# xu-ji/IIC

Measured on AMD Instinct MI355X. Metric: paired-images/sec, STL10 96x96 ClusterNet5g+IID_loss, higher is better.
Workload: dtype bf16; 1 GPU; STL10 96x96 ClusterNet5g IID+ (cluster_sobel.py train step), batch 660 pairs/GPU, 5 sub-heads, k=70, bf16 MFMA convs / fp32 stem+heads+loss, fused HIP Adam; global_batch_pairs=660, input=96x96x1 grey -> sobel 2ch, parallelism=dp1, streams=2, launch=hip-graph replay: 6 linear graph segments, the two views on two streams

## Files before the change

iic_amd/_lib.py:

```python
import ctypes
import os
from ctypes import POINTER, Structure, c_double, c_float, c_int, c_int32, c_long, c_longlong, c_void_p

_HERE = os.path.dirname(os.path.abspath(__file__))
HAS_HOOKS = os.environ.get("IIC_HIP_LIB", "") == "dbg"
LIB_PATH = os.path.join(_HERE, "libiic_hip_dbg.so" if HAS_HOOKS else "libiic_hip.so")

IIC_MAX_TAPS = 32
IIC_STAT_STRIPES = 32


class ConvGeom(Structure):
  _fields_ = [
    ("N", c_int32), ("MY", c_int32), ("MX", c_int32),
    ("in_Hp", c_int32), ("in_Wp", c_int32), ("Cin", c_int32),
    ("sy", c_int32), ("sx", c_int32), ("oy", c_int32), ("ox", c_int32),
    ("out_Hp", c_int32), ("out_Wp", c_int32), ("Cout", c_int32),
    ("ty", c_int32), ("tx", c_int32), ("py", c_int32), ("px", c_int32),
    ("ntaps", c_int32),
    ("tap_off", c_int32 * IIC_MAX_TAPS),
    ("tap_w", c_int32 * IIC_MAX_TAPS),
    ("NP", c_int32),
    ("NP256", c_int32),
    ("NP64", c_int32),
    ("MP", c_int32),
  ]


_P = c_void_p
_SIGNATURES = {
  "iic_version": (c_int, []),
  "iic_iid_nsplit": (c_int, [c_int]),
  "iic_iid_workspace_bytes": (c_long, [c_int, c_int]),
  "iic_iid_joint_raw": (c_int, [_P, _P, _P, c_int, c_int, c_int, c_long, c_long, c_int, _P]),
  "iic_iid_loss_from_joint": (c_int, [_P, c_int, c_int, c_int, c_double, c_double, _P, _P, _P, _P, _P, _P]),
  "iic_iid_grad": (c_int, [_P, _P, _P, _P, _P, _P, _P, _P, c_int, c_int, c_int, c_long, c_long, _P]),
  "iic_seg_joint_nsplit": (c_int, [c_int, c_int, c_int, c_int]),
  "iic_seg_joint_raw": (c_int, [_P, _P, _P, _P, _P, c_int, c_int, c_int, c_int, c_int, c_int, _P]),
  "iic_seg_loss_from_joint": (c_int, [_P, c_int, c_int, c_int, c_double, c_double, _P, _P, _P, _P, _P, c_int, _P]),
  "iic_seg_grad_workspace_bytes": (c_long, [c_int, c_int]),
  "iic_seg_grad": (c_int, [_P, _P, _P, _P, _P, _P, _P, _P, c_int, c_int, c_int, c_int, c_int, c_int, c_int, _P, _P]),
  "iic_affine_warp_fwd": (c_int, [_P, _P, _P, c_int, c_int, c_int, c_int, c_int, c_int, _P]),
  "iic_affine_warp_bwd": (c_int, [_P, _P, _P, c_int, c_int, c_int, c_int, c_int, c_int, _P]),
  "iic_conv_lds_bytes": (c_long, [POINTER(ConvGeom), c_int]),
  "iic_conv_igemm": (c_int, [POINTER(ConvGeom), _P, _P, _P, _P, _P, _P, c_int, _P]),
  "iic_conv_wgrad_nsplit": (c_int, [POINTER(ConvGeom)]),
  "iic_conv_wgrad": (c_int, [POINTER(ConvGeom), _P, _P, _P, c_int, c_int, _P]),
  "iic_conv_wgrad_reduce": (c_int, [_P, c_int, c_int, c_int, c_int, _P, c_int, _P]),
  "iic_weight_prep": (c_int, [_P, _P, _P, c_int, c_int, c_int, _P]),
  "iic_conv_igemm_frag_supported": (c_int, [POINTER(ConvGeom)]),
  "iic_conv_igemm_frag": (c_int, [POINTER(ConvGeom), _P, _P, _P, _P, _P, _P, c_int, _P]),
  "iic_conv_igemm_red_supported": (c_int, [POINTER(ConvGeom)]),
  "iic_conv_igemm_frag_red": (c_int, [POINTER(ConvGeom), _P, _P, _P, _P, _P, _P, c_int, _P, _P, _P, _P, _P, _P]),
  "iic_weight_prep_frag": (c_int, [_P, _P, c_int, c_int, c_int, c_int, _P]),
  "iic_weight_prep_multi_blocks": (c_long, [c_int, c_int, c_int]),
  "iic_weight_prep_multi": (c_int, [_P, c_int, c_long, _P]),
  "iic_bn_finalize": (c_int, [_P, _P, _P, _P, _P, _P, _P, c_int, c_long, c_long, c_float, c_float, c_int, _P]),
  "iic_stat_bytes": (c_long, [c_int]),
  "iic_bn_running_update": (c_int, [c_int, POINTER(_P), POINTER(_P), POINTER(_P), POINTER(_P), POINTER(c_int),
                                    c_float, _P]),
  "iic_bn_apply": (c_int, [_P, _P, _P, _P, _P, _P, c_int, c_int, c_int, c_int, c_int, c_int, _P]),
  "iic_bn_bwd_reduce": (c_int, [_P, _P, _P, _P, _P, _P, _P, c_int, c_int, c_int, c_int, c_int, _P]),
  "iic_bn_bwd_finalize": (c_int, [_P, _P, _P, _P, _P, _P, c_int, c_long, _P]),
  "iic_bn_bwd_apply": (c_int, [_P, _P, _P, _P, _P, _P, _P, _P, _P, c_int, c_int, c_int, c_int, c_int, _P]),
  "iic_stem_stats": (c_int, [_P, _P, _P, c_int, c_int, c_int, c_int, _P]),
  "iic_stem_apply_pool": (c_int, [_P, _P, _P, _P, c_int, c_int, c_int, c_int, _P]),
  "iic_stem_bwd_reduce": (c_int, [_P, _P, _P, _P, _P, c_int, c_int, c_int, c_int, _P]),
  "iic_stem_wgrad_partial_floats": (c_long, []),
  "iic_stem_bwd_wgrad": (c_int, [_P, _P, _P, _P, _P, _P, _P, c_int, c_int, c_int, c_int, _P]),
  "iic_contingency": (c_int, [_P, _P, c_long, c_int, c_int, _P, _P]),
  "iic_count_equal": (c_int, [_P, _P, c_long, _P, _P]),
  "iic_augment": (c_int, [_P, c_int, c_int, c_int, c_int, _P, _P, c_int, _P, c_int, _P, _P, c_int, _P, _P, c_int, _P, _P]),
  "iic_seg_augment": (c_int, [_P, c_int, c_int, c_int, c_int, _P, _P, _P, _P, c_int, c_int, c_int, c_int, _P, _P, _P, _P,
                              _P, _P]),
  "iic_stem_bwd_fused": (c_int, [_P, _P, _P, _P, _P, _P, POINTER(c_int), c_int, c_int, c_int, c_int, _P]),
  "iic_stem_wgrad_combine": (c_int, [_P, c_int, _P, _P, c_int, _P]),
  "iic_firstconv_fwd": (c_int, [_P, _P, _P, _P, c_int, c_int, c_int, c_int, c_int, c_int, c_int, _P]),
  "iic_firstconv_wgrad_partial_floats": (c_long, []),
  "iic_firstconv_wgrad": (c_int, [_P, _P, _P, _P, c_int, c_int, c_int, c_int, c_int, c_int, c_int, _P]),
  "iic_maxpool2_fwd": (c_int, [_P, _P, c_int, c_int, c_int, c_int, c_int, c_int, _P]),
  "iic_maxpool2_bwd": (c_int, [_P, _P, _P, c_int, c_int, c_int, c_int, c_int, c_int, _P]),
  "iic_bn_relu_maxpool2_fwd": (c_int, [_P, _P, _P, c_int, c_int, c_int, c_int, c_int, c_int, _P]),
  "iic_bn_relu_maxpool2_bwd": (c_int, [_P, _P, _P, _P, c_int, c_int, c_int, c_int, c_int, c_int, _P]),
  "iic_sobel": (c_int, [_P, _P, c_int, c_int, c_int, c_int, c_int, c_int, _P]),
  "iic_avgpool_fwd": (c_int, [_P, _P, c_int, c_int, c_int, c_int, c_int, _P]),
# ... 100 lines not shown
```

iic_amd/archs/cluster.py:

```python
import torch
import torch.nn as nn

from .. import geom as G
from .. import ops

__all__ = ["ClusterNet5g", "ClusterNet5gTwoHead"]

import os
import weakref

from ..dist import SHARD_INPUTS, shard_batch
DEDUP = [int(os.environ.get("IIC_DEDUP", "1"))]
_ASSERTED_REPLICAS = [1]


class replicated(object):

  def __init__(self, r):
    self.r = int(r)

  def __enter__(self):
    self.prev = _ASSERTED_REPLICAS[0]
    _ASSERTED_REPLICAS[0] = self.r
    return self
# ... 194 lines not shown
      dy = ops.pt_alloc(N, H, W, 64, 1, dev)
      ops.bn_bwd_apply(da, None, y, bcoef, dy, N, H, W, 1, 64, mask_coef=coef)
      gf, _ = h.geoms(N, H, W)
      dW = ops.conv_wgrad(gf, xp, dy, 9).view(64, C, 3, 3)
    for t in (dpool, da, dy, xp, y, a):
      ops.POOL.release(t)
    return None, dW, dgamma, dbeta, None


class _BlockFn(torch.autograd.Function):
  @staticmethod
  def forward(ctx, x, w1, g1, b1, w2, g2, b2, wd, gd, bd, blk, chain=None):
    N, Hp, Wp, Cin = x.shape
    H, W = Hp - 2, Wp - 2
    dev = x.device
    h1, h2, hd = blk._h1, blk._h2, blk._hd
    planes = h1.spec.cout
    Ho, Wo = h1.spec.out_size(H), h1.spec.out_size(W)
    cnt = N * Ho * Wo
    need_grad = any(ctx.needs_input_grad)

    def bn_coef(bn, holder, gamma, beta, y_stats):
      rm, rv, nbt = _bn_buffers(bn)
      if _bn_training(bn):
        upd = bn.training
        return ops.bn_finalize(y_stats, gamma.detach(), beta.detach(), rm if upd else None,
                               rv if upd else None, nbt if upd else None, planes, cnt, True)
      return ops.bn_finalize(None, gamma.detach(), beta.detach(), rm, rv, None, planes, cnt, False)

    gf1, _ = h1.geoms(N, H, W)
    gf2, _ = h2.geoms(N, Ho, Wo)
    st1 = h1.stats(dev) if _bn_training(blk.bn1) else None
    y1 = ops.pt_alloc(N, Ho, Wo, planes, 1, dev)
    ops.conv_igemm(gf1, x, h1.weights()[0], y1, stats=st1)
    coef1 = bn_coef(blk.bn1, h1, g1, b1, st1)
    st2 = h2.stats(dev) if _bn_training(blk.bn2) else None
    y2 = ops.pt_alloc(N, Ho, Wo, planes, 1, dev)
    a1 = ops.pt_alloc(N, Ho, Wo, planes, 1, dev)
    ops.bn_apply(y1, coef1, a1, N, Ho, Wo, 1, planes, relu=True)
    ops.conv_igemm(gf2, a1, h2.weights()[0], y2, stats=st2)
    coef2 = bn_coef(blk.bn2, h2, g2, b2, st2)
    out = ops.pt_alloc(N, Ho, Wo, planes, 1, dev)
    yd = coefd = None
    if hd is not None:
      gfd, _ = hd.geoms(N, H, W)
      bnd = blk.downsample[1]
      std = hd.stats(dev) if _bn_training(bnd) else None
      yd = ops.pt_alloc(N, Ho, Wo, planes, 1, dev)
      ops.conv_igemm(gfd, x, hd.weights()[0], yd, stats=std)
      coefd = bn_coef(bnd, hd, gd, bd, std)
      ops.bn_apply(y2, coef2, out, N, Ho, Wo, 1, planes, y2=yd, coef2=coefd, relu=True)
    else:
      ops.bn_apply(y2, coef2, out, N, Ho, Wo, 1, planes, res=x, relu=True)

    if need_grad:
      ctx.blk = blk
      ctx.branch, ctx.pt_dtype = ops.BRANCH[0], ops.PT_DTYPE[0]
      ctx.dims = (N, H, W, Ho, Wo, Cin, planes)
      ctx.bn_batch = (_bn_training(blk.bn1) and _bn_training(blk.bn2))
      ctx.dout_premasked, ctx.mask_dx = blk._dout_premasked, blk._mask_dx
      ctx.dout_prereduced = False
      ctx.red_prev = None
      if chain is not None:
        _, gb1f = h1.geoms(N, H, W)
        if (chain.ctx is not None and FUSE_RED[0] and hd is None and blk._mask_dx and len(gb1f) == 1
            and ops.red_supported(gb1f[0], h1.weights()[1]) and ctx.bn_batch):
          ctx.red_prev = (chain.y2, chain.yd, chain.blk)
          chain.ctx.dout_prereduced = True
        if blk._dout_premasked and ctx.bn_batch:
          chain.ctx, chain.y2, chain.yd, chain.blk = ctx, y2, yd, blk
        else:
          chain.ctx = None
      ctx.save_for_backward(x, y1, a1, y2, out, yd, coef1, coef2, coefd, g1, g2, gd)
    else:
      if chain is not None:
        chain.ctx = None
      for t in (y1, a1, y2, yd):
        if t is not None:
          ops.POOL.release(t)
    return out

  @ops.branch_backward
# ... 31 lines not shown
      gfd, _ = hd.geoms(N, H, W)
      dWd = ops.conv_wgrad(gfd, x, dyd, 1, use_tr).view(planes, Cin, 1, 1)
    da1 = ops.pt_alloc(N, Ho, Wo, planes, 1, dev)
    s1 = h1.stats(dev, "bwd")
    m_act, m_coef = (None, coef1) if BN_MASK_FROM_Y[0] else (a1, None)
    w2b = h2.weights()[1]
    if FUSE_RED[0] and m_coef is not None and len(gb2) == 1 and ops.red_supported(gb2[0], w2b):
      ops.conv_igemm(gb2[0], dy2, w2b, da1, red=(y1, coef1, s1, None, None))
    else:
      for g in gb2:
        ops.conv_igemm(g, dy2, w2b, da1)
      ops.bn_bwd_reduce(da1, m_act, y1, s1, N, Ho, Wo, 1, planes, mask_coef=m_coef)
    bc1, dg1, db1 = ops.bn_bwd_finalize(s1, g1.detach(), coef1, planes, cnt)
    dy1 = ops.pt_alloc(N, Ho, Wo, planes, 1, dev)
    ops.bn_bwd_apply(da1, m_act, y1, bc1, dy1, N, Ho, Wo, 1, planes, mask_coef=m_coef)

    dW1 = ops.conv_wgrad(gf1, x, dy1, 9, use_tr).view(planes, Cin, 3, 3)
    dx = ops.pt_alloc(N, H, W, Cin, 1, dev)
    mx = x if mask_dx else None
    red_prev = None
    if ctx.red_prev is not None:
      py2, pyd, pblk = ctx.red_prev
      red_prev = (py2, None, pblk._h2.stats(dev, "bwd"), pyd,
                  pblk._hd.stats(dev, "bwd") if pyd is not None else None)
    if hd is None:
      for g in gb1:
        if pre or mask_dx:
          assert pre, "a block that pre-masks its input gradient needs a pre-masked output gradient"
          ops.conv_igemm(g, dy1, h1.weights()[1], dx, res_grad=dout, res_act=mx, premask=True,
                         red=red_prev)
        else:
          ops.conv_igemm(g, dy1, h1.weights()[1], dx, res_grad=dout, res_act=out)
    else:
      for g in gb1:
        ops.conv_igemm(g, dy1, h1.weights()[1], dx, res_act=mx, premask=mask_dx)
      _, gbd = hd.geoms(N, H, W)
      for g in gbd:
        ops.conv_igemm(g, dyd, hd.weights()[1], dx, accumulate=True, res_act=mx, premask=mask_dx)

    for t in (dout, dy2, dyd, da1, dy1, y1, a1, y2, yd, out):
      ops.POOL.release(t)
    return dx, dW1, dg1, db1, dW2, dg2, db2, dWd, dgd, dbd, None, None


APPLY_GENERATION = [0]


class _ApplyCounter(object):
  def _apply(self, fn, *a, **k):
    APPLY_GENERATION[0] += 1
    return super(_ApplyCounter, self)._apply(fn, *a, **k)


class BasicBlock(nn.Module):
  expansion = 1

  def __init__(self, inplanes, planes, stride=1, downsample=None, track_running_stats=None):
    super(BasicBlock, self).__init__()
    assert track_running_stats is not None
    self.conv1 = nn.Conv2d(inplanes, planes, kernel_size=3, stride=stride, padding=1, bias=False)
    self.bn1 = nn.BatchNorm2d(planes, track_running_stats=track_running_stats)
    self.conv2 = nn.Conv2d(planes, planes, kernel_size=3, stride=1, padding=1, bias=False)
    self.bn2 = nn.BatchNorm2d(planes, track_running_stats=track_running_stats)
    self.downsample = downsample
    self.stride = stride
    self._h1 = _ConvHolder(self.conv1)
    self._h2 = _ConvHolder(self.conv2)
    self._hd = _ConvHolder(downsample[0]) if downsample is not None else None
    self._use_tr = True
    self._dout_premasked = False
    self._mask_dx = False
# ... 241 lines not shown
```

iic_amd/csrc/conv_igemm_bd.hip:

```cpp
#include "common.h"
#include "conv_tile.h"
#include "../../include/iic_hip.h"

__device__ __forceinline__ void bd_bload(u32x4& d, const unsigned char* p) {
  asm volatile("global_load_dwordx4 %0, %1, off" : "=v"(d) : "v"(p) : "memory");
}
template <int N>
__device__ __forceinline__ void bd_bwait(u32x4& d) {
  asm volatile("s_waitcnt vmcnt(%1)" : "+v"(d) : "i"(N) : "memory");
}

struct bd_blk {
  int bw, bh, nbx, nby;
  int PW, npix, mul;
};

#define BD_BM 256
#define BD_BN 128
#define BD_THREADS 256
#define BD_PROF_SLOTS 16
#ifndef BD_STORE_UB
#define BD_STORE_UB 8
#endif

template <bool GATHER, int ABL, int MS, int RED, int WN = 2>
__device__ __forceinline__ void bd_tile(
    const iic_conv_geom& g, const bf16_t* __restrict__ in, const unsigned char* __restrict__ wfrag,
    bf16_t* __restrict__ out, float* __restrict__ stats, const bf16_t* __restrict__ res_grad,
    const bf16_t* __restrict__ res_act, int accumulate, int lds_a_bytes,
    const bf16_t* __restrict__ red_y, const float* __restrict__ red_coef,
    const bf16_t* __restrict__ red_y2, float* __restrict__ red_stats, float* __restrict__ red_stats2,
    unsigned long long* __restrict__ prof, int blk_in_class, int nwg_class, const bd_blk& B) {
  constexpr int BNT = WN * 64, NWM = 4 / WN;
  constexpr bool CANBLK = !GATHER && MS * 32 * (4 / WN) == 256;
  const bool blk = CANBLK && B.bw > 0;
  constexpr int CLD = BNT + 8;
  constexpr bool PROF = (ABL & 128) != 0;
  constexpr bool NEWORD = (ABL & 256) == 0;
  constexpr bool SWZ = (ABL & 512) == 0;
  unsigned long long t_stamp[8];
  unsigned long long t_bsum = 0, t_b0 = 0;
  int t_nb = 0;
  if (PROF) t_stamp[0] = __builtin_readcyclecounter();
  constexpr int BM = MS * 32 * NWM, WR = MS * 32;
  extern __shared__ __attribute__((aligned(16))) unsigned char smem_raw[];
  unsigned char* sA = smem_raw;
  int* s_pin = reinterpret_cast<int*>(smem_raw + lds_a_bytes);
  int* s_pout = s_pin + BM;
  float* s_red = reinterpret_cast<float*>(s_pout + BM);
  unsigned char* s_key = reinterpret_cast<unsigned char*>(s_red + NWM * 2 * BNT);
  bf16_t* sC = reinterpret_cast<bf16_t*>(smem_raw);

  const int tid = threadIdx.x, lane = tid & 63;
  const int wave = __builtin_amdgcn_readfirstlane(tid >> 6);
  const int wm = WN == 2 ? wave >> 1 : wave, wn = WN == 2 ? wave & 1 : 0;
  const int l31 = lane & 31, g5 = lane >> 5;

  const int nt = g.Cout / BNT;
  const int tix = xcd_tile_index(blk_in_class, nwg_class);
  const int mtile = tix / nt, ntile = tix - mtile * nt;
  const int n0 = ntile * BNT;
  const int m0 = mtile * BM;
  const int in_pixels = g.N * g.in_Hp * g.in_Wp;

  int v_tapoff = g.tap_off[lane & (IIC_MAX_TAPS - 1)];
// ... 29 lines not shown
  const int keyw = blk ? B.PW : g.in_Wp;
  const int jskip = blk ? B.PW - B.bw
                        : ((!GATHER && g.sx == 1 && ((g.in_Wp - g.MX) & 1) == 0) ? g.in_Wp - g.MX : 0);
  auto dense_of = [&](int p) { return p - jskip * (p / keyw); };
  int arow[MS];
  int drow[MS];
#pragma unroll
  for (int ms = 0; ms < MS; ++ms) {
    const int row = wm * WR + ms * 32 + l31;
    const int pr = GATHER ? row : (s_pin[row] - p_lo);
    arow[ms] = SWZ ? pr : pr * ROWB + g5 * 16;
    drow[ms] = (SWZ && !GATHER) ? dense_of(s_pin[row]) : pr;
  }
  if (!GATHER && jskip != 0) {
    for (int r = tid; r < npix; r += BD_THREADS) s_key[r] = (unsigned char)((dense_of(p_lo + r) >> 1) & 7);
    __syncthreads();
  }
  const int v_tapd = v_tapoff - jskip * (v_tapoff / keyw);
  const int nblk = (npix * 128 + 1023) >> 10;
  auto dma_patch = [&](int c0) {
    for (int kb = wave; kb < nblk; kb += BD_THREADS / 64) {
      const int q = kb * 64 + lane;
      const int r = q >> 3;
      const int ls = (q & 7) ^ (GATHER ? ((r >> 1) & 7)
                                       : (jskip != 0 ? (int)s_key[r < npix ? r : npix - 1]
                                                     : (((p_lo + r) >> 1) & 7)));
      long p = GATHER ? (long)s_pin[r < BM ? r : BM - 1] : (long)p_lo + r;
      if (blk) {
        const int rc = r < npix ? r : npix - 1;
        const int py = (rc * B.mul) >> 16;
        p = (long)blk_glo + py * g.in_Wp + (rc - py * B.PW);
      }
      p = p < in_pixels ? p : in_pixels - 1;
      __builtin_amdgcn_global_load_lds(
          (const __attribute__((address_space(1))) void*)(in + (p * g.Cin + c0 + ls * 8)),
          (__attribute__((address_space(3))) void*)(sA + kb * 1024), 16, 0, 0);
    }
    asm volatile("s_waitcnt vmcnt(0)" ::: "memory");
  };
  auto a_base = [&](int R, int D) { return R * 128 + (((g5 ^ (D >> 1)) & 1) << 4); };
  auto a_kk = [&](int D) { return ((D >> 2) & 3) << 5; };

  f32x16 acc[MS][2];
#pragma unroll
  for (int ms = 0; ms < MS; ++ms)
#pragma unroll
    for (int ns = 0; ns < 2; ++ns)
#pragma unroll
      for (int r = 0; r < 16; ++r) acc[ms][ns][r] = 0.f;

  const int nchunks = g.Cin >> 6;
  const int ntaps = g.ntaps;
  const int NIT = nchunks * ntaps;
  const long frag_it = (long)(g.Cout >> 5) * 4096;
  const unsigned char* wb0 = wfrag + (long)((n0 + wn * 64) >> 5) * 4096 + lane * 16;
  auto frag_ptr = [&](int tap, int chunk) {
    const int tw = __builtin_amdgcn_readlane(v_tapw, tap);
    return wb0 + ((long)tw * nchunks + chunk) * frag_it;
  };

  if (PROF) t_stamp[1] = __builtin_readcyclecounter();
  u32x4 Bc[4][2];
  {
    const unsigned char* p = frag_ptr(0, 0);
#pragma unroll
    for (int ks = 0; ks < 4; ++ks)
#pragma unroll
      for (int ns = 0; ns < 2; ++ns)
        if (NEWORD) bd_bload(Bc[ks][ns], p + ns * 4096 + ks * 1024);
        else Bc[ks][ns] = *reinterpret_cast<const u32x4*>(p + ns * 4096 + ks * 1024);
  }
  dma_patch(0);
  __syncthreads();
  if (PROF) t_stamp[2] = __builtin_readcyclecounter();

  int tap = 0, chunk = 0;
  bf16x8 a[2][MS];
  int pcur[MS], kcur[MS];
#pragma unroll
  for (int ms = 0; ms < MS; ++ms) {
    const int t0 = GATHER ? 0 : __builtin_amdgcn_readlane(v_tapoff, 0);
    if (SWZ) {
      const int R = arow[ms] + t0;
      const int D = drow[ms] + (GATHER ? 0 : __builtin_amdgcn_readlane(v_tapd, 0));
      pcur[ms] = a_base(R, D);
      kcur[ms] = a_kk(D);
      a[0][ms] = *reinterpret_cast<const bf16x8*>(sA + pcur[ms] + kcur[ms]);
    } else {
      pcur[ms] = arow[ms] + t0 * ROWB;
// ... 163 lines not shown
  __syncthreads();
  if (PROF) t_stamp[4] = __builtin_readcyclecounter();
  TileRed tr;
  if (RED) tile_red_zero(tr);
  if (!(ABL & 32))
    igemm_store_tile<BNT, BM, BD_THREADS, 8, RED, (BM == 256 ? BD_STORE_UB : 4)>(sC, s_pout, out, res_grad, res_act, accumulate,
                                                                 g.Cout, n0, tid, red_y, red_coef, red_y2, &tr);
  if (RED)
    igemm_red_finish<BNT, BD_THREADS, RED>(tr, reinterpret_cast<float*>(smem_raw), red_stats, red_stats2,
                                             g.Cout, n0, tid);
  if (PROF && prof && tid == 0) {
    unsigned long long* q = prof + (long)blockIdx.x * BD_PROF_SLOTS;
    const unsigned long long t_end = __builtin_readcyclecounter();
    q[0] = t_stamp[0]; q[1] = t_stamp[1]; q[2] = t_stamp[2]; q[3] = t_stamp[3]; q[4] = t_stamp[4];
    q[5] = t_end; q[6] = t_bsum; q[7] = (unsigned long long)t_nb;
    q[8] = (unsigned long long)__builtin_amdgcn_s_getreg((32 - 1) << 11 | 0 << 6 | 4)
           | ((unsigned long long)__builtin_amdgcn_s_getreg((4 - 1) << 11 | 0 << 6 | 20) << 32);
    q[9] = (unsigned long long)tix;
    q[10] = __builtin_amdgcn_s_memrealtime();
  }
}

template <bool GATHER, int ABL, int MS, int RED, int WN = 2>
__global__ __launch_bounds__(BD_THREADS, ((MS == 4 || WN == 1) ? 2 : 3)) void conv_igemm_bd_kernel(
    const iic_conv_geom g, const bf16_t* __restrict__ in, const unsigned char* __restrict__ wfrag,
    bf16_t* __restrict__ out, float* __restrict__ stats, const bf16_t* __restrict__ res_grad,
    const bf16_t* __restrict__ res_act, int accumulate, int num_mtiles, int lds_a_bytes,
    const bf16_t* __restrict__ red_y, const float* __restrict__ red_coef,
    const bf16_t* __restrict__ red_y2, float* __restrict__ red_stats, float* __restrict__ red_stats2,
    unsigned long long* __restrict__ prof, const bd_blk B) {
  bd_tile<GATHER, ABL, MS, RED, WN>(g, in, wfrag, out, stats, res_grad, res_act, accumulate, lds_a_bytes, red_y,
                                    red_coef, red_y2, red_stats, red_stats2, prof, (int)blockIdx.x,
                                    num_mtiles * (g.Cout / (WN * 64)), B);
}

__global__ void weight_prep_frag_kernel(const float* __restrict__ w, bf16_t* __restrict__ o, int Co,
                                        int Ci, int T, int mode) {
  const int Nn = mode ? Ci : Co, Kk = mode ? Co : Ci;
  const int n32 = Nn >> 5, nchunks = Kk >> 6;
  const long total = (long)T * Co * Ci;
  for (long i = (long)blockIdx.x * blockDim.x + threadIdx.x; i < total;
       i += (long)gridDim.x * blockDim.x) {
    const int e = (int)(i & 7), lane = (int)((i >> 3) & 63), ks = (int)((i >> 9) & 3);
    long r = i >> 11;
    const int j = (int)(r % n32);
    r /= n32;
    const int kc = (int)(r % nchunks), t = (int)(r / nchunks);
    const int n = j * 32 + (lane & 31), k = kc * 64 + ks * 16 + (lane >> 5) * 8 + e;
    const int co = mode ? k : n, ci = mode ? n : k;
    o[i] = f32_to_bf16(w[((long)co * Ci + ci) * T + t]);
  }
}

int iic_p64_supported(const iic_conv_geom* g);
int iic_p64_launch(const iic_conv_geom* g, const void* in, const void* wfrag, void* out, float* stats,
                   const void* res_grad, const void* res_act, int accumulate, const void* red_y,
                   const float* red_coef, const void* red_y2, float* red_stats, float* red_stats2,
                   void* stream);
int iic_pw_supported(const iic_conv_geom* g);
int iic_pw_launch(const iic_conv_geom* g, const void* in, const void* wfrag, void* out, float* stats,
                  const void* res_grad, const void* res_act, int accumulate, const void* red_y,
                  const float* red_coef, const void* red_y2, float* red_stats, float* red_stats2, void* stream);
IIC_SWITCH(g_p64_enabled, 1, iic_debug_enable_p64)
IIC_SWITCH(g_p64_red, 0, iic_debug_p64_red)

extern "C" {
// ... 196 lines not shown
    if ((AB_ != 0 && AB_ != 128 && AB_ != 256) || GA_ || red == 0) {                             \
      if (red != 0) return IIC_ERR_UNSUPPORTED;                                                  \
      BD_LAUNCH4(GA_, AB_, MS_, 0);                                                              \
    } else if (red == 1) BD_LAUNCH4(false, (AB_ == 128 || AB_ == 256 ? AB_ : 0), MS_, 1);        \
    else BD_LAUNCH4(false, (AB_ == 128 || AB_ == 256 ? AB_ : 0), MS_, 2);                        \
  } while (0)
#define BD_LAUNCH(GA_, AB_)                                                                       \
  do {                                                                                           \
    if (ms == 4) BD_LAUNCH3(GA_, AB_, 4); else BD_LAUNCH3(GA_, AB_, 2);                          \
  } while (0)
  if (g->ntaps == 1) BD_LAUNCH(true, 0);
  else switch (iic_debug_get_ablate()) {
#ifdef IIC_BD_ABLATIONS
    case 1: BD_LAUNCH(false, 1); break;
    case 2: BD_LAUNCH(false, 2); break;
    case 3: BD_LAUNCH(false, 3); break;
    case 4: BD_LAUNCH(false, 4); break;
    case 7: BD_LAUNCH(false, 7); break;
    case 15: BD_LAUNCH(false, 15); break;
    case 16: BD_LAUNCH(false, 16); break;
    case 31: BD_LAUNCH(false, 31); break;
    case 32: BD_LAUNCH(false, 32); break;
    case 64: BD_LAUNCH(false, 64); break;
    case 96: BD_LAUNCH(false, 96); break;
    case 128: BD_LAUNCH(false, 128); break;
    case 256: BD_LAUNCH(false, 256); break;
    case 512: BD_LAUNCH(false, 512); break;
#endif
    default: BD_LAUNCH(false, 0); break;
  }
  return iic_launch_status();
}

__global__ __launch_bounds__(256) void weight_prep_multi_kernel(const iic_weight_prep_job* __restrict__ jobs,
                                                                int njobs) {
  int lo = 0, hi = njobs - 1;
  while (lo < hi) {
    const int mid = (lo + hi + 1) >> 1;
    if ((long long)blockIdx.x >= jobs[mid].first_block) lo = mid; else hi = mid - 1;
  }
  const iic_weight_prep_job j = jobs[lo];
  const float* __restrict__ w = j.w;
  bf16_t* __restrict__ o = reinterpret_cast<bf16_t*>(j.out);
  const int Co = j.Cout, Ci = j.Cin, T = j.T, mode = j.mode;
  const long total = (long)T * Co * Ci;
  const long nblk = (total + 2047) >> 11;
  const long b = (long)blockIdx.x - j.first_block;
  if (b >= nblk) return;
  for (long i = b * 256 + threadIdx.x; i < total; i += nblk * 256) {
    if (mode <= 1) {
      const int Nn = mode ? Ci : Co, Kk = mode ? Co : Ci;
      const int n32 = Nn >> 5, nchunks = Kk >> 6;
      const int e = (int)(i & 7), lane = (int)((i >> 3) & 63), ks = (int)((i >> 9) & 3);
      long r = i >> 11;
      const int jj = (int)(r % n32);
      r /= n32;
      const int kc = (int)(r % nchunks), t = (int)(r / nchunks);
      const int n = jj * 32 + (lane & 31), k = kc * 64 + ks * 16 + (lane >> 5) * 8 + e;
      const int co = mode ? k : n, ci = mode ? n : k;
      o[i] = f32_to_bf16(w[((long)co * Ci + ci) * T + t]);
    } else if (mode == 2) {
      const int ci = (int)(i % Ci);
      const long r = i / Ci;
      const int co = (int)(r % Co), t = (int)(r / Co);
      o[i] = f32_to_bf16(w[((long)co * Ci + ci) * T + t]);
    } else {
// ... 32 lines not shown
```

iic_amd/ops.py:

```python
import ctypes
import os
import threading
import weakref

import torch

from . import _lib
from ._lib import IIC_STAT_STRIPES, check, lib, ptr, stream_ptr

BF16 = torch.bfloat16
F32 = torch.float32


class BranchContext(object):
  __slots__ = ("branch", "streams", "proxies", "deferred_running", "pending_join", "branch_main", "no_proxy_branches",
               "capture_proxies", "solo_first")

  def __init__(self):
    self.branch = 0
    self.streams = {}
    self.proxies = {}
    self.deferred_running = []
    self.pending_join = []
    self.branch_main = None
# ... 533 lines not shown


def conv_igemm(g, x_pt, w_t, out_pt, stats=None, res_grad=None, res_act=None, accumulate=False,
               premask=False, red=None):
  acc = (ACC_ADD if accumulate else 0) | (ACC_PREMASK if premask else 0)
  if x_pt.dtype == F32:
    assert isinstance(w_t, WOperand) and red is None and out_pt.dtype == F32
    w = w_t.pw.w
    check(lib().iic_f32_conv(ctypes.byref(g), ptr(x_pt), ptr(w), w.shape[2] * w.shape[3], 1 if w_t.bwd else 0,
                             ptr(out_pt), ptr(stats), ptr(res_grad), ptr(res_act), acc, stream_ptr()),
          "iic_f32_conv")
    return out_pt
  if red is not None:
    assert red_supported(g, w_t), "fused reduction needs the weights-direct kernel"
    ry, rcoef, rsums, ry2, rsums2 = red
    check(lib().iic_conv_igemm_frag_red(ctypes.byref(g), ptr(x_pt), ptr(w_t.pw.frag(w_t.bwd)),
                                        ptr(out_pt), ptr(stats), ptr(res_grad), ptr(res_act), acc,
                                        ptr(ry), ptr(rcoef), ptr(ry2), ptr(rsums), ptr(rsums2),
                                        stream_ptr()), "iic_conv_igemm_frag_red")
    return out_pt
  if isinstance(w_t, WOperand):
    if frag_supported(g):
      check(lib().iic_conv_igemm_frag(ctypes.byref(g), ptr(x_pt), ptr(w_t.pw.frag(w_t.bwd)),
                                      ptr(out_pt), ptr(stats), ptr(res_grad), ptr(res_act), acc,
                                      stream_ptr()), "iic_conv_igemm_frag")
      return out_pt
    w_t = w_t.pw.rows(w_t.bwd)
  check(lib().iic_conv_igemm(ctypes.byref(g), ptr(x_pt), ptr(w_t), ptr(out_pt), ptr(stats),
                             ptr(res_grad), ptr(res_act), acc, stream_ptr()),
        "iic_conv_igemm")
  return out_pt


_WG_PART = {}


def _conv_wgrad_launch(g, x_pt, dy_pt, wtaps, use_tr, out, accumulate, ns, key):
  need = ns * g.ntaps * g.Cout * g.Cin
  part = _WG_PART.get(key)
  if part is None or part.numel() < need:
    part = torch.empty(max(need, 1 << 22), dtype=F32, device=x_pt.device)
    _WG_PART[key] = part
  check(lib().iic_conv_wgrad(ctypes.byref(g), ptr(x_pt), ptr(dy_pt), ptr(part), ns,
                             1 if use_tr else 0, stream_ptr()), "iic_conv_wgrad")
  check(lib().iic_conv_wgrad_reduce(ptr(part), ns, wtaps, g.Cout, g.Cin, ptr(out),
                                    1 if accumulate else 0, stream_ptr()), "iic_conv_wgrad_reduce")


def conv_wgrad(g, x_pt, dy_pt, wtaps, use_tr=True, out=None, accumulate=False, nsplit=None):
  if x_pt.dtype == F32:
    if out is None:
      out = torch.empty((g.Cout, g.Cin, wtaps), dtype=F32, device=x_pt.device)
    check(lib().iic_f32_wgrad(ctypes.byref(g), ptr(x_pt), ptr(dy_pt), ptr(out), wtaps, 1 if accumulate else 0,
                              stream_ptr()), "iic_f32_wgrad")
    return out
  ns = int(nsplit) if nsplit else lib().iic_conv_wgrad_nsplit(ctypes.byref(g))
  if out is None:
    out = torch.empty((g.Cout, g.Cin, wtaps), dtype=F32, device=x_pt.device)
  assert g.ntaps == wtaps, "wgrad geometry must list every weight tap once"
  _conv_wgrad_launch(g, x_pt, dy_pt, wtaps, use_tr, out, accumulate, ns, (str(x_pt.device), BRANCH[0]))
  return out


BN_EPS = 1e-5
BN_MOMENTUM = 0.1

# ... 255 lines not shown
```

include/iic_hip.h:

```cpp
#ifndef IIC_HIP_H
#define IIC_HIP_H
#include <stdint.h>
#ifdef __cplusplus
extern "C" {
#endif
#if defined(__GNUC__) || defined(__clang__)
#pragma GCC visibility push(default)
#endif

#define IIC_OK 0
#define IIC_ERR_ARG (-1)
#define IIC_ERR_LAUNCH (-2)
#define IIC_ERR_UNSUPPORTED (-3)

int iic_version(void);

int iic_iid_nsplit(int bn);
long iic_iid_workspace_bytes(int H, int k);
int iic_iid_joint_raw(const float* z, const float* zt, float* partials, int H, int bn, int k,
                      long head_stride, long ld, int nsplit, void* stream);
int iic_iid_loss_from_joint(const float* partials, int nparts, int H, int k, double lamb,
                            double eps, void* workspace, float* loss, float* loss_no_lamb,
                            float* dR_loss, float* dR_loss_no_lamb, void* stream);
int iic_iid_grad(const float* z, const float* zt, const float* dR_loss,
// ... 29 lines not shown
  int32_t tap_off[IIC_MAX_TAPS];
  int32_t tap_w[IIC_MAX_TAPS];
  int32_t NP;
  int32_t NP256;
  int32_t NP64;
  int32_t MP;
} iic_conv_geom;

long iic_conv_lds_bytes(const iic_conv_geom* g, int BN);
#define IIC_STAT_STRIPES 32
long iic_stat_bytes(int C);
#define IIC_ACC_ADD 1
#define IIC_ACC_PREMASK 2
int iic_conv_igemm(const iic_conv_geom* g, const void* in, const void* w, void* out,
                   float* stats, const void* res_grad, const void* res_act, int accumulate,
                   void* stream);
int iic_conv_wgrad_nsplit(const iic_conv_geom* g);
int iic_conv_wgrad(const iic_conv_geom* g, const void* x, const void* dy, float* partials,
                   int nsplit, int use_tr, void* stream);
int iic_conv_wgrad_reduce(const float* partials, int nsplit, int T, int Cout, int Cin, float* dW,
                          int accumulate, void* stream);
int iic_weight_prep(const float* w_oihw, void* w_fwd, void* w_bwd, int Cout, int Cin, int T,
                    void* stream);

int iic_conv_igemm_frag_supported(const iic_conv_geom* g);
int iic_conv_igemm_frag(const iic_conv_geom* g, const void* in, const void* w_frag, void* out,
                        float* stats, const void* res_grad, const void* res_act, int accumulate,
                        void* stream);
int iic_conv_igemm_red_supported(const iic_conv_geom* g);
int iic_conv_igemm_frag_red(const iic_conv_geom* g, const void* in, const void* w_frag, void* out,
                            float* stats, const void* res_grad, const void* res_act, int accumulate,
                            const void* red_y, const float* red_coef, const void* red_y2,
                            float* red_stats, float* red_stats2, void* stream);
int iic_weight_prep_frag(const float* w_oihw, void* w_frag, int Cout, int Cin, int T, int bwd,
                         void* stream);
typedef struct iic_weight_prep_job {
  const float* w;
  void* out;
  long long first_block;
  int32_t Cout, Cin, T, mode;
} iic_weight_prep_job;
long iic_weight_prep_multi_blocks(int Cout, int Cin, int T);
int iic_weight_prep_multi(const iic_weight_prep_job* jobs_dev, int njobs, long total_blocks, void* stream);

int iic_bn_finalize(float* stats, const float* gamma, const float* beta, float* running_mean,
                    float* running_var, long long* num_batches_tracked, float* coef, int C,
                    long count, long unbiased_count, float eps, float momentum, int training,
                    void* stream);
int iic_bn_running_update(int n, const float* const* coef, float* const* running_mean,
                          float* const* running_var, long long* const* num_batches_tracked,
                          const int* C, float momentum, void* stream);
int iic_bn_apply(const void* y, const float* coef, const void* res, const void* y2,
                 const float* coef2, void* out, int N, int H, int W, int P, int C, int relu,
                 void* stream);
int iic_bn_bwd_reduce(const void* dout, const void* act, const void* y, const void* y2,
                      float* sums, float* sums2, const float* mask_coef, int N, int H, int W, int P,
                      int C, void* stream);
int iic_bn_bwd_finalize(float* sums, const float* gamma, const float* coef, float* bcoef,
                        float* dgamma, float* dbeta, int C, long count, void* stream);
int iic_bn_bwd_apply(const void* dout, const void* act, const void* y, const float* bcoef,
                     void* dy, const void* y2, const float* bcoef2, void* dy2,
                     const float* mask_coef, int N, int H, int W, int P, int C, void* stream);

int iic_stem_stats(const float* x, const float* w, float* stats, int N, int Cin, int H, int W,
                   void* stream);
int iic_stem_apply_pool(const float* x, const float* w, const float* coef, void* out_pt, int N,
// ... 131 lines not shown
```

Before: 18900 paired-images/sec.

## Fuse residual downsample 1x1 conv with first 3x3 conv in forward and backward-data

In the forward pass of downsampling residual blocks, one kernel now runs the 3x3 conv tile and then the 1x1 shortcut conv tile on the same workgroup, so the shared input tile is likely still cache-resident and one launch disappears. In backward-data, the 1x1 shortcut's contribution is folded into the matching one-tap sub-GEMM of the 3x3 dx by extending its K dimension over a second input and weight set. This removes the separate accumulate pass that re-read and re-wrote dx. The cost is extra kernel variants with narrower support checks, longer serial tiles per workgroup, and possible occupancy changes.

After: 18820 paired-images/sec. No clear change (-0.4%).

```diff
diff --git a/iic_amd/_lib.py b/iic_amd/_lib.py
--- a/iic_amd/_lib.py
+++ b/iic_amd/_lib.py
@@ -51,6 +51,10 @@
   "iic_conv_igemm_frag_supported": (c_int, [POINTER(ConvGeom)]),
   "iic_conv_igemm_frag": (c_int, [POINTER(ConvGeom), _P, _P, _P, _P, _P, _P, c_int, _P]),
   "iic_conv_igemm_red_supported": (c_int, [POINTER(ConvGeom)]),
+  "iic_conv_igemm_ds_supported": (c_int, [POINTER(ConvGeom), POINTER(ConvGeom)]),
+  "iic_conv_igemm_frag_ds": (c_int, [POINTER(ConvGeom), POINTER(ConvGeom), _P, _P, _P, _P, _P, _P, _P, _P]),
+  "iic_conv_igemm_kx_supported": (c_int, [POINTER(ConvGeom), POINTER(ConvGeom)]),
+  "iic_conv_igemm_frag_kx": (c_int, [POINTER(ConvGeom), POINTER(ConvGeom), _P, _P, _P, _P, _P, _P, c_int, _P]),
   "iic_conv_igemm_frag_red": (c_int, [POINTER(ConvGeom), _P, _P, _P, _P, _P, _P, c_int, _P, _P, _P, _P, _P, _P]),
   "iic_weight_prep_frag": (c_int, [_P, _P, c_int, c_int, c_int, c_int, _P]),
   "iic_weight_prep_multi_blocks": (c_long, [c_int, c_int, c_int]),
diff --git a/iic_amd/archs/cluster.py b/iic_amd/archs/cluster.py
--- a/iic_amd/archs/cluster.py
+++ b/iic_amd/archs/cluster.py
@@ -250,7 +250,17 @@
     gf2, _ = h2.geoms(N, Ho, Wo)
     st1 = h1.stats(dev) if _bn_training(blk.bn1) else None
     y1 = ops.pt_alloc(N, Ho, Wo, planes, 1, dev)
-    ops.conv_igemm(gf1, x, h1.weights()[0], y1, stats=st1)
+    yd = std = None
+    fuse_ds = False
+    if hd is not None:
+      gfd, _ = hd.geoms(N, H, W)
+      fuse_ds = ops.conv_ds_supported(gf1, gfd, h1.weights()[0], hd.weights()[0])
+    if fuse_ds:
+      std = hd.stats(dev) if _bn_training(blk.downsample[1]) else None
+      yd = ops.pt_alloc(N, Ho, Wo, planes, 1, dev)
+      ops.conv_igemm_ds(gf1, gfd, x, h1.weights()[0], hd.weights()[0], y1, yd, stats1=st1, statsd=std)
+    else:
+      ops.conv_igemm(gf1, x, h1.weights()[0], y1, stats=st1)
     coef1 = bn_coef(blk.bn1, h1, g1, b1, st1)
     st2 = h2.stats(dev) if _bn_training(blk.bn2) else None
     y2 = ops.pt_alloc(N, Ho, Wo, planes, 1, dev)
@@ -259,13 +269,13 @@
     ops.conv_igemm(gf2, a1, h2.weights()[0], y2, stats=st2)
     coef2 = bn_coef(blk.bn2, h2, g2, b2, st2)
     out = ops.pt_alloc(N, Ho, Wo, planes, 1, dev)
-    yd = coefd = None
+    coefd = None
     if hd is not None:
-      gfd, _ = hd.geoms(N, H, W)
       bnd = blk.downsample[1]
-      std = hd.stats(dev) if _bn_training(bnd) else None
-      yd = ops.pt_alloc(N, Ho, Wo, planes, 1, dev)
-      ops.conv_igemm(gfd, x, hd.weights()[0], yd, stats=std)
+      if not fuse_ds:
+        std = hd.stats(dev) if _bn_training(bnd) else None
+        yd = ops.pt_alloc(N, Ho, Wo, planes, 1, dev)
+        ops.conv_igemm(gfd, x, hd.weights()[0], yd, stats=std)
       coefd = bn_coef(bnd, hd, gd, bd, std)
       ops.bn_apply(y2, coef2, out, N, Ho, Wo, 1, planes, y2=yd, coef2=coefd, relu=True)
     else:
@@ -363,11 +373,19 @@
         else:
           ops.conv_igemm(g, dy1, h1.weights()[1], dx, res_grad=dout, res_act=out)
     else:
+      _, gbd = hd.geoms(N, H, W)
+      w1b, wdb = h1.weights()[1], hd.weights()[1]
+      kx = None
+      if len(gbd) == 1:
+        kx = next((g for g in gb1 if ops.conv_kx_supported(g, gbd[0], w1b, wdb)), None)
       for g in gb1:
-        ops.conv_igemm(g, dy1, h1.weights()[1], dx, res_act=mx, premask=mask_dx)
-      _, gbd = hd.geoms(N, H, W)
-      for g in gbd:
-        ops.conv_igemm(g, dyd, hd.weights()[1], dx, accumulate=True, res_act=mx, premask=mask_dx)
+        if g is kx:
+          ops.conv_igemm_kx(g, gbd[0], dy1, w1b, dyd, wdb, dx, res_act=mx, premask=mask_dx)
+        else:
+          ops.conv_igemm(g, dy1, w1b, dx, res_act=mx, premask=mask_dx)
+      if kx is None:
+        for g in gbd:
+          ops.conv_igemm(g, dyd, wdb, dx, accumulate=True, res_act=mx, premask=mask_dx)
 
     for t in (dout, dy2, dyd, da1, dy1, y1, a1, y2, yd, out):
       ops.POOL.release(t)
diff --git a/iic_amd/csrc/conv_igemm_bd.hip b/iic_amd/csrc/conv_igemm_bd.hip
--- a/iic_amd/csrc/conv_igemm_bd.hip
+++ b/iic_amd/csrc/conv_igemm_bd.hip
@@ -23,14 +23,16 @@
 #define BD_STORE_UB 8
 #endif
 
-template <bool GATHER, int ABL, int MS, int RED, int WN = 2>
+template <bool GATHER, int ABL, int MS, int RED, int WN = 2, bool KX = false>
 __device__ __forceinline__ void bd_tile(
     const iic_conv_geom& g, const bf16_t* __restrict__ in, const unsigned char* __restrict__ wfrag,
     bf16_t* __restrict__ out, float* __restrict__ stats, const bf16_t* __restrict__ res_grad,
     const bf16_t* __restrict__ res_act, int accumulate, int lds_a_bytes,
     const bf16_t* __restrict__ red_y, const float* __restrict__ red_coef,
     const bf16_t* __restrict__ red_y2, float* __restrict__ red_stats, float* __restrict__ red_stats2,
-    unsigned long long* __restrict__ prof, int blk_in_class, int nwg_class, const bd_blk& B) {
+    unsigned long long* __restrict__ prof, int blk_in_class, int nwg_class, const bd_blk& B,
+    const bf16_t* __restrict__ in2 = nullptr, const unsigned char* __restrict__ wfrag2 = nullptr) {
+  static_assert(!KX || GATHER, "the K-extension is built for the one-tap gather tiles");
   constexpr int BNT = WN * 64, NWM = 4 / WN;
   constexpr bool CANBLK = !GATHER && MS * 32 * (4 / WN) == 256;
   const bool blk = CANBLK && B.bw > 0;
@@ -126,8 +128,9 @@
         p = (long)blk_glo + py * g.in_Wp + (rc - py * B.PW);
       }
       p = p < in_pixels ? p : in_pixels - 1;
+      const bf16_t* src = (KX && c0 >= g.Cin) ? in2 - g.Cin : in;
       __builtin_amdgcn_global_load_lds(
-          (const __attribute__((address_space(1))) void*)(in + (p * g.Cin + c0 + ls * 8)),
+          (const __attribute__((address_space(1))) void*)(src + (p * g.Cin + c0 + ls * 8)),
           (__attribute__((address_space(3))) void*)(sA + kb * 1024), 16, 0, 0);
     }
     asm volatile("s_waitcnt vmcnt(0)" ::: "memory");
@@ -145,10 +148,12 @@
 
   const int nchunks = g.Cin >> 6;
   const int ntaps = g.ntaps;
-  const int NIT = nchunks * ntaps;
+  const int NIT = (KX ? 2 : 1) * nchunks * ntaps;
   const long frag_it = (long)(g.Cout >> 5) * 4096;
   const unsigned char* wb0 = wfrag + (long)((n0 + wn * 64) >> 5) * 4096 + lane * 16;
+  const unsigned char* wb1 = KX ? wfrag2 + (long)((n0 + wn * 64) >> 5) * 4096 + lane * 16 : nullptr;
   auto frag_ptr = [&](int tap, int chunk) {
+    if (KX && chunk >= nchunks) return wb1 + (long)(chunk - nchunks) * frag_it;
     const int tw = __builtin_amdgcn_readlane(v_tapw, tap);
     return wb0 + ((long)tw * nchunks + chunk) * frag_it;
   };
@@ -378,6 +383,31 @@
   bd_tile<GATHER, ABL, MS, RED, WN>(g, in, wfrag, out, stats, res_grad, res_act, accumulate, lds_a_bytes, red_y,
                                     red_coef, red_y2, red_stats, red_stats2, prof, (int)blockIdx.x,
                                     num_mtiles * (g.Cout / (WN * 64)), B);
+}
+
+template <int MS>
+__global__ __launch_bounds__(BD_THREADS, (MS == 4 ? 2 : 3)) void conv_igemm_bd_ds_kernel(
+    const iic_conv_geom g1, const iic_conv_geom gd, const bf16_t* __restrict__ in,
+    const unsigned char* __restrict__ wfrag1, const unsigned char* __restrict__ wfragd, bf16_t* __restrict__ out1,
+    bf16_t* __restrict__ outd, float* __restrict__ stats1, float* __restrict__ statsd, int num_mtiles, int lds_a1,
+    int lds_ad) {
+  const bd_blk B0 = {0, 0, 0, 0, 0, 0, 0};
+  const int nwg = num_mtiles * (g1.Cout / BD_BN);
+  bd_tile<false, 0, MS, 0>(g1, in, wfrag1, out1, stats1, nullptr, nullptr, 0, lds_a1, nullptr, nullptr, nullptr, nullptr,
+                           nullptr, nullptr, (int)blockIdx.x, nwg, B0);
+  __syncthreads();
+  bd_tile<true, 0, MS, 0>(gd, in, wfragd, outd, statsd, nullptr, nullptr, 0, lds_ad, nullptr, nullptr, nullptr, nullptr,
+                          nullptr, nullptr, (int)blockIdx.x, nwg, B0);
+}
+
+__global__ __launch_bounds__(BD_THREADS, 2) void conv_igemm_bd_kx_kernel(
+    const iic_conv_geom g, const bf16_t* __restrict__ in, const unsigned char* __restrict__ wfrag,
+    const bf16_t* __restrict__ in2, const unsigned char* __restrict__ wfrag2, bf16_t* __restrict__ out,
+    const bf16_t* __restrict__ res_act, int accumulate, int num_mtiles, int lds_a_bytes) {
+  const bd_blk B0 = {0, 0, 0, 0, 0, 0, 0};
+  bd_tile<true, 0, 4, 0, 2, true>(g, in, wfrag, out, nullptr, nullptr, res_act, accumulate, lds_a_bytes, nullptr, nullptr,
+                                  nullptr, nullptr, nullptr, nullptr, (int)blockIdx.x, num_mtiles * (g.Cout / BD_BN), B0,
+                                  in2, wfrag2);
 }
 
 __global__ void weight_prep_frag_kernel(const float* __restrict__ w, bf16_t* __restrict__ o, int Co,
@@ -640,6 +670,86 @@
   return iic_launch_status();
 }
 
+static bool ds_same_rows(const iic_conv_geom* a, const iic_conv_geom* b) {
+  return a->N == b->N && a->MY == b->MY && a->MX == b->MX && a->in_Hp == b->in_Hp && a->in_Wp == b->in_Wp &&
+         a->Cin == b->Cin && a->sy == b->sy && a->sx == b->sx && a->out_Hp == b->out_Hp && a->out_Wp == b->out_Wp &&
+         a->Cout == b->Cout && a->ty == b->ty && a->tx == b->tx && a->py == b->py && a->px == b->px && a->MP == b->MP;
+}
+static bool ds_plain_bd(const iic_conv_geom* g) {
+  if (!iic_conv_igemm_frag_supported(g) || g->Cout % BD_BN != 0 || g->Cin % 64 != 0) return false;
+  if (g_p64_enabled && iic_p64_supported(g)) return false;
+  if (iic_debug_get_ablate() != 0 || g_bd_ms != 0 || iic_pw_supported(g)) return false;
+  bd_blk B;
+  if (bd_block_config(g, &B, 2)) return false;
+  const long M = igemm_rows_host(g);
+  return M > 0 && M < (1L << 31) && (long)g->N * g->in_Hp * g->in_Wp < (1L << 31) && bd_pick_ms(g) != 0;
+}
+
+int iic_conv_igemm_ds_supported(const iic_conv_geom* g1, const iic_conv_geom* gd) {
+  if (!g1 || !gd || g1->ntaps < 2 || gd->ntaps != 1 || !ds_same_rows(g1, gd)) return 0;
+  if (!ds_plain_bd(g1) || !ds_plain_bd(gd)) return 0;
+  const long pd = (long)(gd->oy - g1->oy) * gd->in_Wp + (gd->ox - g1->ox) + gd->tap_off[0];
+  bool centre = false;
+  for (int t = 0; t < g1->ntaps; ++t) centre = centre || g1->tap_off[t] == pd;
+  return centre ? 1 : 0;
+}
+
+int iic_conv_igemm_frag_ds(const iic_conv_geom* g1, const iic_conv_geom* gd, const void* in, const void* wfrag1,
+                           const void* wfragd, void* out1, void* outd, float* stats1, float* statsd, void* stream) {
+  if (!g1 || !gd || !in || !wfrag1 || !wfragd || !out1 || !outd) return IIC_ERR_ARG;
+  if (!iic_conv_igemm_ds_supported(g1, gd)) return IIC_ERR_UNSUPPORTED;
+  const int ms = bd_pick_ms(g1);
+  const long M = igemm_rows_host(g1);
+  const int bm = ms * 64;
+  const int mt = (int)((M + bm - 1) / bm);
+  const int grid = mt * (g1->Cout / BD_BN);
+  const int la1 = (int)bd_lds_a(g1, ms), lad = (int)bd_lds_a(gd, ms);
+  const long l1 = bd_lds_total(g1, ms), ld = bd_lds_total(gd, ms);
+  const long lds = l1 > ld ? l1 : ld;
+  hipStream_t s = (hipStream_t)stream;
+#define BD_LAUNCH_DS(MS_)                                                                                     \
+  do {                                                                                                       \
+    static bool attr = false;                                                                                \
+    if (!attr) {                                                                                             \
+      (void)hipFuncSetAttribute(reinterpret_cast<const void*>(&conv_igemm_bd_ds_kernel<MS_>),                \
+                                hipFuncAttributeMaxDynamicSharedMemorySize, 160 * 1024);                     \
+      attr = true;                                                                                           \
+    }                                                                                                        \
+    hipLaunchKernelGGL((conv_igemm_bd_ds_kernel<MS_>), dim3(grid), dim3(BD_THREADS), lds, s, *g1, *gd,       \
+                       (const bf16_t*)in, (const unsigned char*)wfrag1, (const unsigned char*)wfragd,        \
+                       (bf16_t*)out1, (bf16_t*)outd, stats1, statsd, mt, la1, lad);                          \
+  } while (0)
+  if (ms == 4) BD_LAUNCH_DS(4); else BD_LAUNCH_DS(2);
+  return iic_launch_status();
+}
+
+int iic_conv_igemm_kx_supported(const iic_conv_geom* g, const iic_conv_geom* g2) {
+  if (!g || !g2 || g->ntaps != 1 || g2->ntaps != 1 || !ds_same_rows(g, g2)) return 0;
+  if (g->oy != g2->oy || g->ox != g2->ox || g->tap_off[0] != g2->tap_off[0] || g2->tap_w[0] != 0) return 0;
+  return (ds_plain_bd(g) && bd_pick_ms(g) == 4) ? 1 : 0;
+}
+
+int iic_conv_igemm_frag_kx(const iic_conv_geom* g, const iic_conv_geom* g2, const void* in, const void* wfrag,
+                           const void* in2, const void* wfrag2, void* out, const void* res_act, int accumulate,
+                           void* stream) {
+  if (!g || !g2 || !in || !wfrag || !in2 || !wfrag2 || !out) return IIC_ERR_ARG;
+  if (!(accumulate & IIC_ACC_PREMASK) && res_act != nullptr) return IIC_ERR_ARG;
+  if (!iic_conv_igemm_kx_supported(g, g2)) return IIC_ERR_UNSUPPORTED;
+  const long M = igemm_rows_host(g);
+  const int mt = (int)((M + 255) / 256);
+  static bool attr = false;
+  if (!attr) {
+    (void)hipFuncSetAttribute(reinterpret_cast<const void*>(&conv_igemm_bd_kx_kernel),
+                              hipFuncAttributeMaxDynamicSharedMemorySize, 160 * 1024);
+    attr = true;
+  }
+  hipLaunchKernelGGL(conv_igemm_bd_kx_kernel, dim3(mt * (g->Cout / BD_BN)), dim3(BD_THREADS), bd_lds_total(g, 4),
+                     (hipStream_t)stream, *g, (const bf16_t*)in, (const unsigned char*)wfrag, (const bf16_t*)in2,
+                     (const unsigned char*)wfrag2, (bf16_t*)out, (const bf16_t*)res_act, accumulate, mt,
+                     (int)bd_lds_a(g, 4));
+  return iic_launch_status();
+}
+
 __global__ __launch_bounds__(256) void weight_prep_multi_kernel(const iic_weight_prep_job* __restrict__ jobs,
                                                                 int njobs) {
   int lo = 0, hi = njobs - 1;
diff --git a/iic_amd/ops.py b/iic_amd/ops.py
--- a/iic_amd/ops.py
+++ b/iic_amd/ops.py
@@ -589,6 +589,45 @@
   return out_pt
 
 
+FUSE_DS = [os.environ.get("IIC_FUSE_DS", "1") != "0"]
+
+
+def _pair_supported(query, tag, ga, gb, wa, wb):
+  if not FUSE_DS[0] or PT_DTYPE[0] is not BF16 or not (isinstance(wa, WOperand) and isinstance(wb, WOperand)):
+    return False
+  if not (frag_supported(ga) and frag_supported(gb)):
+    return False
+  cache = ga.__dict__.setdefault(tag, {})
+  ent = cache.get(id(gb))
+  if ent is None:
+    ent = cache[id(gb)] = (gb, bool(query(ctypes.byref(ga), ctypes.byref(gb))))
+  return ent[1]
+
+
+def conv_ds_supported(g1, gd, w1, wd):
+  return _pair_supported(lib().iic_conv_igemm_ds_supported, "_ds_ok", g1, gd, w1, wd)
+
+
+def conv_igemm_ds(g1, gd, x_pt, w1, wd, y1_pt, yd_pt, stats1=None, statsd=None):
+  assert conv_ds_supported(g1, gd, w1, wd), "fused shortcut forward: unsupported geometry pair"
+  check(lib().iic_conv_igemm_frag_ds(ctypes.byref(g1), ctypes.byref(gd), ptr(x_pt), ptr(w1.pw.frag(w1.bwd)),
+                                     ptr(wd.pw.frag(wd.bwd)), ptr(y1_pt), ptr(yd_pt), ptr(stats1), ptr(statsd),
+                                     stream_ptr()), "iic_conv_igemm_frag_ds")
+  return y1_pt, yd_pt
+
+
+def conv_kx_supported(g, g2, w, w2):
+  return _pair_supported(lib().iic_conv_igemm_kx_supported, "_kx_ok", g, g2, w, w2)
+
+
+def conv_igemm_kx(g, g2, dy_pt, w, dy2_pt, w2, out_pt, res_act=None, premask=False):
+  assert conv_kx_supported(g, g2, w, w2), "fused shortcut backward-data: unsupported geometry pair"
+  check(lib().iic_conv_igemm_frag_kx(ctypes.byref(g), ctypes.byref(g2), ptr(dy_pt), ptr(w.pw.frag(w.bwd)),
+                                     ptr(dy2_pt), ptr(w2.pw.frag(w2.bwd)), ptr(out_pt), ptr(res_act),
+                                     ACC_PREMASK if premask else 0, stream_ptr()), "iic_conv_igemm_frag_kx")
+  return out_pt
+
+
 _WG_PART = {}
 
 
diff --git a/include/iic_hip.h b/include/iic_hip.h
--- a/include/iic_hip.h
+++ b/include/iic_hip.h
@@ -85,6 +85,13 @@
                             float* stats, const void* res_grad, const void* res_act, int accumulate,
                             const void* red_y, const float* red_coef, const void* red_y2,
                             float* red_stats, float* red_stats2, void* stream);
+int iic_conv_igemm_ds_supported(const iic_conv_geom* g1, const iic_conv_geom* gd);
+int iic_conv_igemm_frag_ds(const iic_conv_geom* g1, const iic_conv_geom* gd, const void* in, const void* w_frag1,
+                           const void* w_fragd, void* out1, void* outd, float* stats1, float* statsd, void* stream);
+int iic_conv_igemm_kx_supported(const iic_conv_geom* g, const iic_conv_geom* g2);
+int iic_conv_igemm_frag_kx(const iic_conv_geom* g, const iic_conv_geom* g2, const void* in, const void* w_frag,
+                           const void* in2, const void* w_frag2, void* out, const void* res_act, int accumulate,
+                           void* stream);
 int iic_weight_prep_frag(const float* w_oihw, void* w_frag, int Cout, int Cin, int T, int bwd,
                          void* stream);
 typedef struct iic_weight_prep_job {
```
